# jixinya/EAMM

Hardware: AMD Instinct MI355X
Metric: 256x256 frames/sec (dense-motion + generator forward) (higher is better)
Workload: dtype f32; 1 GPU; 256x256, 10 keypoints, batch=16 synthetic frames per GPU per step, source encoded once per clip (BASELINE.json configs[2]); parallelism=frame-sharded x1

## Files before the change

eamm_amd/csrc/api_common.h:

```cpp
#pragma once
#include "../../include/eamm_hip.h"
#include "kernels.h"

#include <algorithm>
#include <cmath>
#include <cstdarg>
#include <cstdio>
#include <cstdlib>
#include <cstring>
#include <map>
#include <string>
#include <vector>

namespace eamm {

inline thread_local std::string g_create_error;

namespace {

struct HostTensor {
    std::vector<int64_t> shape;
    std::vector<float> data;
    size_t numel() const {
        size_t n = 1;
// ... 170 lines not shown

enum LayerMode { MODE_PLAIN = 0, MODE_PHASE = 1, MODE_ROWSPLIT = 2, MODE_PHASES = 3 };

int upload_bias(CtxBase* c, float** dst, const std::vector<float>& b, size_t n) {
    std::vector<float> pad(n, 0.f);
    std::copy(b.begin(), b.end(), pad.begin());
    return upload(c, dst, pad);
}

int upload_conv_image(CtxBase* c, float** dst, const HostConv& f, const int* map, int cin_packed, int BN, LayerMode mode,
                      bool swizzle) {
    const bool phase = mode == MODE_PHASE || mode == MODE_PHASES;
    std::vector<float> packed(conv_packed_elems(phase ? 4 : f.kh * f.kw, cin_packed, f.Cout, BN, phase ? 4 : 1));
    if (mode == MODE_PHASES)
        conv_pack_phases_host(f.w.data(), f.Cout, f.Cin, map, cin_packed, BN, swizzle, packed.data());
    else
        conv_pack_host(f.w.data(), f.Cout, f.Cin, f.kh, f.kw, map, cin_packed, BN, phase, swizzle, packed.data());
    return upload(c, dst, packed);
}

int pack_conv(CtxBase* c, const HostConv& f, const int* map, int C0_packed, int C1_packed, LayerMode mode, int dma_cfg,
              ConvLayer* L, int BN = 0) {
    const bool phase = mode == MODE_PHASE || mode == MODE_PHASES;
    L->kh = f.kh;
    L->kw = f.kw;
    L->phase = phase;
    L->C0 = C0_packed;
    L->C1 = C1_packed;
    L->Cout = f.Cout;
    L->BM = 128;
    L->BN = BN ? BN : conv_tile_n(f.Cout);
    L->dma_cfg = dma_cfg;
    if (dma_cfg > 0 && !conv_dma_tile(dma_cfg, &L->BM, &L->BN)) return fail(c, EAMM_ERR_ARG, "unknown dma tile %d", dma_cfg);
    L->ntiles = (f.Cout + L->BN - 1) / L->BN;
    L->nchunks = (phase ? 4 : f.kh * f.kw) * ((C0_packed + C1_packed) / CONV_BK);
    if (int rc = upload_conv_image(c, &L->w, f, map, C0_packed + C1_packed, L->BN, mode, dma_cfg > 0)) return rc;
    return upload_bias(c, &L->bias, f.b, (size_t)L->ntiles * L->BN);
}

int pack_patch(CtxBase* c, const HostConv& f, const int* map, int C0_packed, int C1_packed, bool poly, PatchLayer* P) {
    const int cin_packed = C0_packed + C1_packed;
    P->C0 = C0_packed;
    P->C1 = C1_packed;
    P->Cout = f.Cout;
    std::vector<float> packed(poly ? patch_poly_packed_elems(cin_packed, f.Cout) : patch_packed_elems(cin_packed, f.Cout));
    if (poly)
        patch_poly_pack_host(f.w.data(), f.Cout, f.Cin, map, cin_packed, packed.data());
    else
        patch_pack_host(f.w.data(), f.Cout, f.Cin, map, cin_packed, packed.data());
    if (int rc = upload(c, poly ? &P->w_poly : &P->w, packed)) return rc;
    return upload_bias(c, &P->bias, f.b, (size_t)((f.Cout + 63) / 64) * 64);
}

int pack_wino(CtxBase* c, const HostConv& f, int tile, WinoLayer* L) {
    L->Cin = f.Cin;
    L->Cout = f.Cout;
    L->tile = tile;
    L->BN = tile == 4 ? 64 : 128;
    L->ntiles = (f.Cout + L->BN - 1) / L->BN;
    std::vector<float> packed(tile == 4 ? wino4_packed_elems(f.Cout, f.Cin, L->BN) : wino_packed_elems(f.Cout, f.Cin, L->BN));
    if (tile == 4)
        wino4_pack_host(f.w.data(), f.Cout, f.Cin, L->BN, packed.data());
    else
        wino_pack_host(f.w.data(), f.Cout, f.Cin, L->BN, packed.data());
    if (int rc = upload(c, &L->u, packed)) return rc;
    return upload_bias(c, &L->bias, f.b, (size_t)L->ntiles * L->BN);
}

int build_layer(CtxBase* c, const std::vector<FoldSpec>& parts, int ks, int C0_real, int C0_packed, int C1_real,
                int C1_packed, ConvLayer* L, LayerMode mode = MODE_PLAIN, std::vector<float>* row_bias = nullptr,
                int dma_cfg = 0, float** w_swizzled = nullptr, int w_swizzled_bn = 0) {
    if (mode != MODE_PLAIN && mode != MODE_ROWSPLIT) return fail(c, EAMM_ERR_ARG, "build_layer: plain or row-split layers only");
    HostConv f;
    if (int rc = fold_conv(c, parts, ks, C0_real + C1_real, &f)) return rc;
    if (mode == MODE_ROWSPLIT) {
        std::vector<float> rb = to_rowsplit(&f);
        if (row_bias) row_bias->swap(rb);
    }
    const std::vector<int> map = channel_map(C0_real, C0_packed, C1_real, C1_packed);
    if (int rc = pack_conv(c, f, map.data(), C0_packed, C1_packed, MODE_PLAIN, dma_cfg, L)) return rc;
    if (!w_swizzled) return EAMM_OK;
    return upload_conv_image(c, w_swizzled, f, map.data(), C0_packed + C1_packed, w_swizzled_bn ? w_swizzled_bn : L->BN,
                             MODE_PLAIN, true);
}

int build_set(CtxBase* c, const std::vector<FoldSpec>& parts, int C0_real, int C0_packed, int C1_real, int C1_packed,
              LayerSet* S, LayerMode mode) {
    HostConv f;
    int rc = fold_conv(c, parts, 3, C0_real + C1_real, &f);
    if (rc) return rc;
    const std::vector<int> map = channel_map(C0_real, C0_packed, C1_real, C1_packed);
    if ((rc = pack_conv(c, f, map.data(), C0_packed, C1_packed, mode, 0, &S->base))) return rc;
    const int Cout = S->base.Cout;
    int cfg = 0;
    if (Cout % 256 == 0) cfg = c->dma_cfg_n256;
    else if (Cout % 128 == 0) cfg = c->dma_cfg_n128;
    else if (Cout == 64) cfg = c->dma_cfg_n64;
    if (cfg > 0 && c->dma_min_m >= 0) {
        if ((rc = pack_conv(c, f, map.data(), C0_packed, C1_packed, mode, cfg, &S->dma))) return rc;
        S->has_dma = true;
        if (S->dma.BN == 128 && c->skinny_max_m > 0) {
            S->skinny32 = S->dma;
            S->skinny64 = S->dma;
            S->skinny32.dma_cfg = 4;
            S->skinny64.dma_cfg = 5;
            conv_dma_tile(4, &S->skinny32.BM, &S->skinny32.BN);
            conv_dma_tile(5, &S->skinny64.BM, &S->skinny64.BN);
            S->has_skinny = true;
        }
        if (Cout % 256 == 0 && cfg != 1 && c->big_min_m >= 0) {
            if ((rc = pack_conv(c, f, map.data(), C0_packed, C1_packed, mode, 1, &S->big))) return rc;
            S->has_big = true;
        }
    }
    if (mode == MODE_PHASE && parts.size() == 1 && !parts[0].norm.empty() && (Cout & 3) == 0 && c->patch_min_blocks >= 0) {
        if ((rc = pack_patch(c, f, map.data(), C0_packed, C1_packed, c->patch_poly != 0, &S->patch))) return rc;
        S->has_patch = true;
    }
    return 0;
}

size_t set_partial_elems(const LayerSet& S, size_t M) {
    size_t n = conv_plan(S.base, (int)M).partial_elems;
    if (S.has_dma) n = std::max(n, conv_plan(S.dma, (int)M).partial_elems);
    if (S.has_big) n = std::max(n, conv_plan(S.big, (int)M).partial_elems);
    if (S.has_skinny) n = std::max({n, conv_plan(S.skinny32, (int)M).partial_elems, conv_plan(S.skinny64, (int)M).partial_elems});
    return n;
}

int build_wino(CtxBase* c, const std::string& conv, const std::string& norm, int C, WinoLayer* L, int tile = 2) {
    HostConv f;
    if (int rc = fold_conv(c, {{conv, norm}}, 3, C, &f)) return rc;
    if (f.Cout != C) return fail(c, EAMM_ERR_KEY, "%s mis-shaped for the Winograd path", conv.c_str());
    return pack_wino(c, f, tile, L);
}

int build_wino4_rect(CtxBase* c, const std::string& conv, const std::string& norm, int Cin_real, int Cin_packed, WinoLayer* L) {
    if (Cin_packed < Cin_real || Cin_packed % 64) return fail(c, EAMM_ERR_KEY, "%s mis-shaped for the Winograd path", conv.c_str());
    HostConv f;
    if (int rc = fold_conv(c, {{conv, norm}}, 3, Cin_real, &f)) return rc;
    HostConv p = f;
    p.Cin = Cin_packed;
    p.w.assign((size_t)f.Cout * Cin_packed * 9, 0.f);
    for (int o = 0; o < f.Cout; ++o)
        std::copy_n(f.w.begin() + (size_t)o * Cin_real * 9, (size_t)Cin_real * 9, p.w.begin() + (size_t)o * Cin_packed * 9);
    return pack_wino(c, p, 4, L);
}

const ConvLayer& pick(const CtxBase* c, const LayerSet& S, size_t M) {
    if (S.has_skinny && M <= (size_t)c->skinny_max_m) return M <= 32 ? S.skinny32 : S.skinny64;
    if (S.has_big && M >= (size_t)c->big_min_m) return S.big;
    return (S.has_dma && M >= (size_t)c->dma_min_m) ? S.dma : S.base;
}

int launch_up(CtxBase* c, const LayerSet& S, const ConvIO& io, hipStream_t s) {
    if (S.has_patch) {
        int cus = 256;
        (void)hipDeviceGetAttribute(&cus, hipDeviceAttributeMultiprocessorCount, c->device);
        int splits = 1;
        if (S.patch.w_poly) {
            splits = patch_poly_splits(S.patch, io.B, io.Hin, io.Win, c->patch_split_max, cus);
            if ((size_t)splits * io.B * 4 * io.Hin * io.Win * S.patch.Cout > io.partial_cap) splits = 1;
        }
        const int blocks = ((io.Hin + 15) / 16) * ((io.Win + 15) / 16) * io.B * ((S.patch.Cout + 31) / 32) * splits;
        if (blocks >= c->patch_min_blocks && io.Hin >= 16 && io.Win >= 16 && io.act == ACT_RELU && !io.resid && !io.out2 && !io.pool && !io.nchw) {
            if (S.patch.w_poly)
                HIP_TRY(c, patch_poly_launch(S.patch, io.in0, io.in1, io.B, io.Hin, io.Win, io.act, io.out, s, splits, io.partial,
                                             io.partial_cap));
            else
                HIP_TRY(c, patch_phase_launch(S.patch, io.in0, io.in1, io.B, io.Hin, io.Win, io.act, io.out, s));
            return EAMM_OK;
        }
    }
    HIP_TRY(c, conv_launch(pick(c, S, (size_t)io.B * io.Hin * io.Win), io, s));
    return EAMM_OK;
}

int env_int(const char* name, int dflt) { return (int)knob_int(name, dflt); }

int round_up(int v, int m) { return (v + m - 1) / m * m; }

bool is_pow2(int v) { return v > 0 && (v & (v - 1)) == 0; }


inline void read_tile_knobs(CtxBase* c) {
    c->dma_min_m = env_int("EAMM_DMA_MIN_M", c->dma_min_m);
    c->big_min_m = env_int("EAMM_BIG_MIN_M", c->big_min_m);
    c->patch_poly = env_int("EAMM_PATCH_POLY", c->patch_poly);
    c->dma_cfg_n256 = env_int("EAMM_DMA_CFG_N256", c->dma_cfg_n256);
    c->dma_cfg_n128 = env_int("EAMM_DMA_CFG_N128", c->dma_cfg_n128);
    c->dma_cfg_n64 = env_int("EAMM_DMA_CFG_N64", c->dma_cfg_n64);
    c->patch_min_blocks = env_int("EAMM_PATCH_MIN_BLOCKS", c->patch_min_blocks);
    c->patch_split_max = env_int("EAMM_PATCH_SPLIT_MAX", c->patch_split_max);
    c->skinny_max_m = env_int("EAMM_SKINNY_MAX_M", c->skinny_max_m);
}

inline void free_owned(CtxBase* c) {
    DeviceGuard guard(c->device);
    (void)hipDeviceSynchronize();
// ... 38 lines not shown
```

eamm_amd/csrc/conv_winograd4.hip:

```cpp
#include "conv_common.h"

#include <algorithm>
#include <cstdlib>

namespace eamm {

typedef __attribute__((address_space(3))) void* lds_ptr_t;
typedef float f32x4_t __attribute__((ext_vector_type(4)));

template <int VEC> struct vec_of;
template <> struct vec_of<1> { typedef float type; };
template <> struct vec_of<2> { typedef float type __attribute__((ext_vector_type(2))); };
template <> struct vec_of<4> { typedef float type __attribute__((ext_vector_type(4))); };

template <typename T> __device__ __forceinline__ T vfma(float a, T x, T y);
template <> __device__ __forceinline__ float vfma<float>(float a, float x, float y) { return fmaf(a, x, y); }
template <> __device__ __forceinline__ vec_of<2>::type vfma(float a, vec_of<2>::type x, vec_of<2>::type y) {
    vec_of<2>::type r;
    r[0] = fmaf(a, x[0], y[0]); r[1] = fmaf(a, x[1], y[1]);
    return r;
}
template <> __device__ __forceinline__ vec_of<4>::type vfma(float a, vec_of<4>::type x, vec_of<4>::type y) {
    vec_of<4>::type r;
    r[0] = fmaf(a, x[0], y[0]); r[1] = fmaf(a, x[1], y[1]); r[2] = fmaf(a, x[2], y[2]); r[3] = fmaf(a, x[3], y[3]);
    return r;
}
template <typename T> __device__ __forceinline__ T vrelu_affine(T v, T sc, T sh);
template <> __device__ __forceinline__ float vrelu_affine<float>(float v, float sc, float sh) { return fmaxf(fmaf(v, sc, sh), 0.f); }
template <> __device__ __forceinline__ vec_of<2>::type vrelu_affine(vec_of<2>::type v, vec_of<2>::type sc, vec_of<2>::type sh) {
    vec_of<2>::type r;
    r[0] = fmaxf(fmaf(v[0], sc[0], sh[0]), 0.f); r[1] = fmaxf(fmaf(v[1], sc[1], sh[1]), 0.f);
    return r;
}
template <> __device__ __forceinline__ vec_of<4>::type vrelu_affine(vec_of<4>::type v, vec_of<4>::type sc, vec_of<4>::type sh) {
    vec_of<4>::type r;
    r[0] = fmaxf(fmaf(v[0], sc[0], sh[0]), 0.f); r[1] = fmaxf(fmaf(v[1], sc[1], sh[1]), 0.f);
    r[2] = fmaxf(fmaf(v[2], sc[2], sh[2]), 0.f); r[3] = fmaxf(fmaf(v[3], sc[3], sh[3]), 0.f);
    return r;
}

template <typename T> __device__ __forceinline__ void bt6(T& d0, T& d1, T& d2, T& d3, T& d4, T& d5) {
    const T s12 = d1 + d2, m12 = d1 - d2;
    const T s34 = d3 + d4, m43 = d4 - d3;
    const T m31 = d3 - d1, m42 = d4 - d2;
    const T t0 = vfma(4.f, d0, vfma(-5.f, d2, d4));
    const T t1 = vfma(-4.f, s12, s34);
    const T t2 = vfma(4.f, m12, m43);
    const T t3 = vfma(2.f, m31, m42);
    const T t4 = vfma(-2.f, m31, m42);
    const T t5 = vfma(4.f, d1, vfma(-5.f, d3, d5));
    d0 = t0; d1 = t1; d2 = t2; d3 = t3; d4 = t4; d5 = t5;
}

template <int VEC>
__global__ __launch_bounds__(256) void wino4_input_transform_kernel(const float* __restrict__ x,
                                                                    const float* __restrict__ s,
// ... 34 lines not shown
            for (int j = 0; j < 6; ++j) d[i][j] = img[(size_t)(yo[i] + xo[j]) * cvn];
#pragma unroll
        for (int i = 0; i < 6; ++i)
#pragma unroll
            for (int j = 0; j < 6; ++j) {
                T v = d[i][j];
                if (s != nullptr) v = vrelu_affine(v, sc, sh);
                d[i][j] = (oky[i] && okx[j]) ? v : T(0.f);
            }
#pragma unroll
        for (int j = 0; j < 6; ++j) bt6(d[0][j], d[1][j], d[2][j], d[3][j], d[4][j], d[5][j]);
        T* out = reinterpret_cast<T*>(V) + q * cvn + cv;
        const size_t plane = Mq * cvn;
#pragma unroll
        for (int i = 0; i < 6; ++i) {
            bt6(d[i][0], d[i][1], d[i][2], d[i][3], d[i][4], d[i][5]);
            if constexpr (VEC == 4) {
                if (by_xcd & 2) {
                    const __amdgpu_buffer_rsrc_t rs = __builtin_amdgcn_make_buffer_rsrc((void*)V, 0, (unsigned)(36 * plane * 16), 0x00020000);
#pragma unroll
                    for (int j = 0; j < 6; ++j)
                        __builtin_amdgcn_raw_buffer_store_b128(__builtin_bit_cast(u32x4, d[i][j]), rs,
                                                               (unsigned)(((size_t)(i * 6 + j) * plane + q * cvn + cv) * 16), 0, 2);
                    continue;
                }
            }
#pragma unroll
            for (int j = 0; j < 6; ++j) out[(size_t)(i * 6 + j) * plane] = d[i][j];
        }
    }
}

struct Wino4Args {
    const float* V;
    const float* U;
    const float* bias;
    unsigned v_bytes, u_bytes;
    int Mq, C, Cout;
    int H, W;
    int mtiles, ntiles;
    int act;
    const float* resid;
    float* out;
    int groups;
    float* zout;
    float* epi_scratch;
};

__constant__ float WINO4_AT[4][8] = {{1.f, 1.f, 1.f, 1.f, 1.f, 0.f, 0.f, 0.f},
                                     {0.f, 1.f, -1.f, 2.f, -2.f, 0.f, 0.f, 0.f},
                                     {0.f, 1.f, 1.f, 4.f, 4.f, 0.f, 0.f, 0.f},
                                     {0.f, 1.f, -1.f, 8.f, -8.f, 1.f, 0.f, 0.f}};

template <int NT, int WM, int WN, int SUB, int NST, int PE, int DBG = 0>
__global__ __launch_bounds__(WM* WN * 64) void wino4_gemm_kernel(const Wino4Args p) {
    constexpr int NW = WM * WN, NTHR = NW * 64;
    constexpr int BM = WM * 16, BN = WN * NT * 16, BK = CONV_BK;
    constexpr int A_STAGE = SUB * BM * BK, B_STAGE = SUB * BN * BK;
    constexpr int A_INSTR = BM / 8 / NW, B_INSTR = BN / 8 / NW;
    constexpr int NPIECE = SUB * (A_INSTR + B_INSTR);
    constexpr bool TRACE = DBG == 8 || DBG == 9;
    static_assert(BM % (8 * NW) == 0 && BN % (8 * NW) == 0, "tile rows must split evenly over the waves");
    static_assert(BK == 32, "two 16-wide K steps per chunk");

    extern __shared__ __attribute__((aligned(16))) float smem[];
    float* const As = smem;
    float* const Bs = smem + NST * A_STAGE;

    const int tid = threadIdx.x;
    const int lane = tid & 63;
    const int wave = __builtin_amdgcn_readfirstlane(tid >> 6);
    const int r16 = lane & 15, g = lane >> 4;
    const int wm = wave / WN, wn = wave % WN;

    const int L = xcd_remap(blockIdx.x, gridDim.x);
    const int ntile = L % p.ntiles;
    const int mtile = (L / p.ntiles) % p.mtiles;
    const int grp = L / (p.ntiles * p.mtiles);
    const int xis_per = 36 / p.groups;
    const int xi0 = grp * xis_per;
    const int mbase = mtile * BM;
    const int cchunks = p.C / BK;
    const int ci_base = xi0 * cchunks;
    const int nsuper = xis_per * cchunks / SUB;

    unsigned arow_off[A_INSTR];
#pragma unroll
    for (int j = 0; j < A_INSTR; ++j) {
        const int row = (wave * A_INSTR + j) * 8 + (lane >> 3);
        const int slot = (lane & 7) ^ ((row >> 1) & 7);
        const int m = mbase + row;
        arow_off[j] = m < p.Mq ? (unsigned)(m * p.C + slot * 4) * 4u : 0xFFFFF000u;
    }
    const unsigned b_lane = (unsigned)lane * 16u;
    const __amdgpu_buffer_rsrc_t rsv = __builtin_amdgcn_make_buffer_rsrc((void*)p.V, 0, p.v_bytes, 0x00020000);
    const __amdgpu_buffer_rsrc_t rsu = __builtin_amdgcn_make_buffer_rsrc((void*)p.U, 0, p.u_bytes, 0x00020000);
    const unsigned plane_bytes = (unsigned)p.Mq * (unsigned)p.C * 4u;
    const unsigned a_wrap = plane_bytes - (unsigned)(cchunks * BK * 4);

    unsigned sa_off = (unsigned)xi0 * plane_bytes;
    unsigned sb_off = (unsigned)((ntile * 36 * cchunks + ci_base) * BN * BK) * 4u +
                      (unsigned)(wave * B_INSTR * 8 * BK) * 4u;
    int dma_cc = 0, n_st = 0;
    auto dma_advance = [&]() {
        dma_cc += SUB;
        sa_off += SUB * BK * 4;
        if (dma_cc == cchunks) {
            dma_cc = 0;
            sa_off += a_wrap;
        }
        sb_off += SUB * BN * BK * 4;
        n_st = n_st + 1 == NST ? 0 : n_st + 1;
    };
    auto dma_piece = [&](auto kc) {
        constexpr int k = decltype(kc)::value;
        constexpr int sub = k / (A_INSTR + B_INSTR), r = k % (A_INSTR + B_INSTR);
        if constexpr (r < A_INSTR) {
            float* dst = As + n_st * A_STAGE + sub * (BM * BK) + (wave * A_INSTR + r) * (8 * BK) - sub * BK;
            const unsigned vo = arow_off[r];
            __builtin_amdgcn_raw_ptr_buffer_load_lds(rsv, (lds_ptr_t)dst, 16, vo, sa_off, sub * BK * 4, DBG == 40 ? 2 : 0);
        } else {
            constexpr int j = r - A_INSTR;
            float* dst = Bs + n_st * B_STAGE + sub * (BN * BK) + (wave * B_INSTR + j) * (8 * BK);
            __builtin_amdgcn_raw_ptr_buffer_load_lds(rsu, (lds_ptr_t)dst, 16, b_lane,
                                                     sb_off + (unsigned)((sub * BN + j * 8) * BK * 4), 0, 0);
        }
    };

    f32x4_t acc[NT];
    f32x4_t Z[4][NT];
    f32x4_t Y[16][NT];
    static_for<NT>([&](auto jc) {
        constexpr int j = decltype(jc)::value;
        static_for<4>([&](auto rc) {
            constexpr int r = decltype(rc)::value;
            acc[j][r] = 0.f;
            static_for<4>([&](auto qc) { Z[decltype(qc)::value][j][r] = 0.f; });
            static_for<16>([&](auto pc) { Y[decltype(pc)::value][j][r] = 0.f; });
        });
    });

    const int sw = (r16 >> 1) & 7;
    constexpr int STEPS = SUB * 2;
    constexpr int MF = 4 * NT;
    constexpr int TOTAL_MF = STEPS * MF;
    static_assert(PE >= 1 && NPIECE * PE <= TOTAL_MF, "DMA pieces must fit in the interval");
    auto compute = [&](int st, auto more_c, auto young_c) {
        constexpr bool MORE = decltype(more_c)::value && DBG != 1 && DBG != 9, YOUNG = decltype(young_c)::value;
        f32x4_t a[2], b[2][NT];
        auto fetch = [&](int step, int buf) {
            const int sub = step >> 1, s = step & 1;
            const int slot = ((4 * s + g) ^ sw) << 2;
            const float* a_base = As + st * A_STAGE + sub * (BM * BK) + (wm * 16 + r16) * BK + slot;
            const float* b_base = Bs + st * B_STAGE + sub * (BN * BK) + (wn * NT * 16 + r16) * BK + slot;
            a[buf] = *reinterpret_cast<const f32x4_t*>(a_base);
#pragma unroll
            for (int j = 0; j < NT; ++j) b[buf][j] = *reinterpret_cast<const f32x4_t*>(b_base + j * 16 * BK);
        };
        fetch(0, 0);
        if constexpr (MORE && YOUNG) static_for<NPIECE>([&](auto kc) { dma_piece(kc); });
        static_for<STEPS>([&](auto sc) {
            constexpr int step = decltype(sc)::value;
            if constexpr (step + 1 < STEPS) fetch(step + 1, (step + 1) & 1);
            __builtin_amdgcn_sched_barrier(0);
            static_for<MF>([&](auto qc) {
                constexpr int q = decltype(qc)::value;
                constexpr int t = q / NT, j = q % NT;
                acc[j] = __builtin_amdgcn_mfma_f32_16x16x4f32(a[step & 1][t], b[step & 1][j][t], acc[j], 0, 0, 0);
                constexpr int gi = step * MF + q;
                if constexpr (MORE && !YOUNG && gi % PE == PE - 1 && gi / PE < NPIECE) {
                    __builtin_amdgcn_sched_barrier(0);
                    dma_piece(std::integral_constant<int, gi / PE>{});
                    __builtin_amdgcn_sched_barrier(0);
                }
            });
        });
    };
    const bool young = wave >= NW / 2;
    auto interval = [&](int st, bool more) {
        if (more) {
            if (young) compute(st, std::true_type{}, std::true_type{});
            else compute(st, std::true_type{}, std::false_type{});
            dma_advance();
        } else {
            compute(st, std::false_type{}, std::false_type{});
        }
    };

    auto fold_x = [&](int j) {
        const float c0 = WINO4_AT[0][j], c1 = WINO4_AT[1][j], c2 = WINO4_AT[2][j], c3 = WINO4_AT[3][j];
        static_for<NT>([&](auto jc) {
            constexpr int jj = decltype(jc)::value;
            static_for<4>([&](auto rc) {
                constexpr int r = decltype(rc)::value;
                const float m = acc[jj][r];
                Z[0][jj][r] = fmaf(c0, m, Z[0][jj][r]);
                Z[1][jj][r] = fmaf(c1, m, Z[1][jj][r]);
                Z[2][jj][r] = fmaf(c2, m, Z[2][jj][r]);
                Z[3][jj][r] = fmaf(c3, m, Z[3][jj][r]);
                acc[jj][r] = 0.f;
            });
        });
    };
    auto fold_y = [&](int i) {
        const float c0 = WINO4_AT[0][i], c1 = WINO4_AT[1][i], c2 = WINO4_AT[2][i], c3 = WINO4_AT[3][i];
        static_for<NT>([&](auto jc) {
            constexpr int jj = decltype(jc)::value;
            static_for<4>([&](auto qc) {
                constexpr int q = decltype(qc)::value;
                static_for<4>([&](auto rc) {
                    constexpr int r = decltype(rc)::value;
                    const float z = Z[q][jj][r];
                    Y[0 + q][jj][r] = fmaf(c0, z, Y[0 + q][jj][r]);
                    Y[4 + q][jj][r] = fmaf(c1, z, Y[4 + q][jj][r]);
                    Y[8 + q][jj][r] = fmaf(c2, z, Y[8 + q][jj][r]);
                    Y[12 + q][jj][r] = fmaf(c3, z, Y[12 + q][jj][r]);
                    Z[q][jj][r] = 0.f;
                });
            });
        });
    };

    auto store_z = [&](int i) {
        static_for<4>([&](auto qc) {
            constexpr int q = decltype(qc)::value;
            static_for<NT>([&](auto jc) {
                constexpr int jj = decltype(jc)::value;
                const int col = ntile * BN + wn * NT * 16 + jj * 16 + r16;
                static_for<4>([&](auto rc) {
                    constexpr int r = decltype(rc)::value;
                    const int row = mbase + wm * 16 + 4 * g + r;
                    if (row < p.Mq && col < p.Cout) p.zout[((size_t)(i * 4 + q) * p.Mq + row) * p.Cout + col] = Z[q][jj][r];
                    Z[q][jj][r] = 0.f;
                });
            });
        });
    };

// ... 125 lines not shown
        const int qx = m % Wq, tq = m / Wq;
        const int qy = tq % Hq, b = tq / Hq;
        const f32x4_t* z = reinterpret_cast<const f32x4_t*>(Z) + idx;
        const f32x4_t bs = reinterpret_cast<const f32x4_t*>(bias)[c4];
        const float lo = act == ACT_RELU ? 0.f : -INFINITY;
        f32x4_t colsum[2];
#pragma unroll
        for (int q = 0; q < 4; ++q) {
            f32x4_t zi[6];
#pragma unroll
            for (int i = 0; i < 6; ++i) zi[i] = z[(size_t)(i * 4 + q) * plane];
            const f32x4_t s12 = zi[1] + zi[2], d12 = zi[1] - zi[2], s34 = zi[3] + zi[4], d34 = zi[3] - zi[4];
            f32x4_t y[4];
            y[0] = zi[0] + s12 + s34;
            y[1] = d12 + 2.f * d34;
            y[2] = s12 + 4.f * s34;
            y[3] = d12 + 8.f * d34 + zi[5];
            f32x4_t r4[4];
            if constexpr (RESID) {
#pragma unroll
                for (int pp = 0; pp < 4; ++pp)
                    r4[pp] = reinterpret_cast<const f32x4_t*>(resid)[(((size_t)(b * H + 4 * qy + pp) * W + 4 * qx + q) * Cout) / 4 + c4];
            }
#pragma unroll
            for (int pp = 0; pp < 4; ++pp) {
                f32x4_t v = y[pp] + bs;
                if constexpr (!POOL) {
                    const size_t o = (((size_t)(b * H + 4 * qy + pp) * W + 4 * qx + q) * Cout) / 4 + c4;
                    if constexpr (RESID) v = v + r4[pp];
                    v[0] = fmaxf(v[0], lo); v[1] = fmaxf(v[1], lo); v[2] = fmaxf(v[2], lo); v[3] = fmaxf(v[3], lo);
                    reinterpret_cast<f32x4_t*>(out)[o] = v;
                } else {
                    v[0] = fmaxf(v[0], lo); v[1] = fmaxf(v[1], lo); v[2] = fmaxf(v[2], lo); v[3] = fmaxf(v[3], lo);
                    y[pp] = v;
                }
            }
            if constexpr (POOL) {
                if ((q & 1) == 0) {
                    colsum[0] = y[0] + y[1];
                    colsum[1] = y[2] + y[3];
                } else {
#pragma unroll
                    for (int py = 0; py < 2; ++py) {
                        const f32x4_t v = 0.25f * (colsum[py] + (y[2 * py] + y[2 * py + 1]));
                        const size_t o = (((size_t)(b * (H >> 1) + 2 * qy + py) * (W >> 1) + 2 * qx + (q >> 1)) * Cout) / 4 + c4;
                        reinterpret_cast<f32x4_t*>(out)[o] = v;
                    }
                }
            }
        }
    }
}

void wino4_pack_host(const float* w, int Cout, int Cin, int BN, float* dst) {
    static const double G[6][3] = {{1.0 / 4, 0, 0},           {-1.0 / 6, -1.0 / 6, -1.0 / 6}, {-1.0 / 6, 1.0 / 6, -1.0 / 6},
                                   {1.0 / 24, 1.0 / 12, 1.0 / 6}, {1.0 / 24, -1.0 / 12, 1.0 / 6},  {0, 0, 1}};
    const int BK = CONV_BK, cch = Cin / BK;
    const int ntiles = (Cout + BN - 1) / BN;
    const size_t total = (size_t)ntiles * 36 * cch * BN * BK;
    for (size_t i = 0; i < total; ++i) dst[i] = 0.f;
    for (int o = 0; o < Cout; ++o) {
        const int nt = o / BN, nl = o % BN;
        for (int c = 0; c < Cin; ++c) {
            const float* gw = w + ((size_t)o * Cin + c) * 9;
            double tmp[6][3];
            for (int i = 0; i < 6; ++i)
                for (int k = 0; k < 3; ++k)
                    tmp[i][k] = G[i][0] * gw[0 * 3 + k] + G[i][1] * gw[1 * 3 + k] + G[i][2] * gw[2 * 3 + k];
            const int cc = c / BK, kl = c % BK;
            const int kk = ((((kl >> 2) ^ ((nl >> 1) & 7)) << 2) | (kl & 3));
            for (int i = 0; i < 6; ++i)
                for (int j = 0; j < 6; ++j) {
                    const double u = tmp[i][0] * G[j][0] + tmp[i][1] * G[j][1] + tmp[i][2] * G[j][2];
                    const int xi = i * 6 + j;
                    dst[(((size_t)nt * 36 * cch + (size_t)xi * cch + cc) * BN + nl) * BK + kk] = (float)u;
                }
        }
    }
}

size_t wino4_packed_elems(int Cout, int Cin, int BN) {
    return (size_t)((Cout + BN - 1) / BN) * 36 * (Cin / CONV_BK) * BN * CONV_BK;
}

hipError_t wino4_transform_launch(const float* x, const float* s, const float* t, int B, int H, int W, int C, float* V,
                                  hipStream_t stream) {
    if ((H & 3) || (W & 3) || (C & 3)) return hipErrorInvalidValue;
    static const int vec_env = [] {
        const int v = (int)knob_int("EAMM_WINO4_TR_VEC", 0);
        return (v == 1 || v == 2 || v == 4) ? v : 0;
    }();
    const int vec = vec_env ? vec_env : ((size_t)B * (H / 4) * (W / 4) * (C / 4) <= 64 * 256 ? 1 : 4);
    const size_t total = (size_t)B * (H / 4) * (W / 4) * (C / vec);
    const int blocks = (int)std::min<size_t>((total + 255) / 256, (size_t)1 << 20);
    static const int xcd = (int)knob_int("EAMM_WINO4_TR_XCD", 3);
    const int remap = ((size_t)blocks * 256 >= total ? (xcd & 1) : 0) | ((36.0 * total * 16 < 4.0e9 && vec == 4) ? (xcd & 2) : 0);
    if (vec == 1)
        hipLaunchKernelGGL(wino4_input_transform_kernel<1>, dim3(blocks), dim3(256), 0, stream, x, s, t, B, H, W, C, V, remap);
    else if (vec == 2)
        hipLaunchKernelGGL(wino4_input_transform_kernel<2>, dim3(blocks), dim3(256), 0, stream, x, s, t, B, H, W, C, V, remap);
    else
        hipLaunchKernelGGL(wino4_input_transform_kernel<4>, dim3(blocks), dim3(256), 0, stream, x, s, t, B, H, W, C, V, remap);
    return hipGetLastError();
}

template <int SUB, int NST, int PE, int DBG = 0, int WM = 4>
static hipError_t wino4_launch_variant(const Wino4Args& a, hipStream_t stream) {
    constexpr int NT = 2, WN = 2;
    constexpr int BM = WM * 16, BN = WN * NT * 16;
    constexpr size_t lds_loop = sizeof(float) * NST * SUB * (BM + BN) * CONV_BK;
    constexpr size_t lds_epi = sizeof(float) * 4 * BM * (BN + 4);
    constexpr size_t lds = lds_loop > lds_epi ? lds_loop : lds_epi;
    static_assert(lds <= 160 * 1024, "LDS budget");
    auto kern = wino4_gemm_kernel<NT, WM, WN, SUB, NST, PE, DBG>;
    static lds_once_mask configured{0};
    if (hipError_t e = ensure_dynamic_lds(kern, lds, &configured); e != hipSuccess) return e;
    note_mfma_flops(2.0 * 36.0 * a.mtiles * BM * (double)a.ntiles * BN * a.C);
    hipLaunchKernelGGL(kern, dim3(a.mtiles * a.ntiles * a.groups), dim3(WM * WN * 64), lds, stream, a);
    return hipGetLastError();
}

hipError_t wino4_gemm_launch(const WinoLayer& L, const float* V, int B, int H, int W, int act, const float* resid,
                             float* out, hipStream_t stream, int variant, int groups, float* zbuf, int pool) {
    constexpr int BM = 64, BN = 64;
    if (pool && (groups == 1 || resid != nullptr)) return hipErrorInvalidValue;
    if (L.tile != 4 || L.BN != BN || (L.Cout & 3) || L.Cin % (2 * CONV_BK) || (H & 3) || (W & 3))
        return hipErrorInvalidValue;
    Wino4Args a{};
    a.V = V;
    a.U = L.u;
    a.bias = L.bias;
    a.Mq = B * (H / 4) * (W / 4);
    a.C = L.Cin;
    a.Cout = L.Cout;
    a.H = H;
    a.W = W;
    a.mtiles = (a.Mq + BM - 1) / BM;
    a.ntiles = L.ntiles;
    static const int narrow_max = (int)knob_int("EAMM_WINO4_NARROW_MAX_BLOCKS", 128);
    const bool narrow = groups == 6 && a.mtiles * a.ntiles * groups <= narrow_max && L.Cin % (4 * CONV_BK) == 0;
    if (narrow) a.mtiles = (a.Mq + 31) / 32;
    a.act = act;
    a.resid = resid;
    a.out = out;
    if (groups != 1 && groups != 2 && groups != 3 && groups != 6) return hipErrorInvalidValue;
    if (groups > 1 && zbuf == nullptr) return hipErrorInvalidValue;
    a.groups = groups;
    a.zout = groups > 1 ? zbuf : nullptr;
#ifdef EAMM_EXPERIMENTS
    a.epi_scratch = (variant == 50 && groups == 1) ? zbuf : nullptr;
    if (variant == 50 && a.epi_scratch == nullptr) variant = 3;
#else
    if (variant == 10 || variant == 16 || variant == 17 || variant == 50) return hipErrorInvalidValue;
#endif
    const size_t vb = (size_t)36 * a.Mq * a.C * sizeof(float), ub = wino4_packed_elems(L.Cout, L.Cin, BN) * sizeof(float);
    if (vb >= 0xFFFFF000ull || ub >= 0xFFFFF000ull) return hipErrorInvalidValue;
    a.v_bytes = (unsigned)vb;
    a.u_bytes = (unsigned)ub;
    const bool sub4 = L.Cin % (4 * CONV_BK) == 0;
    hipError_t e = hipErrorInvalidValue;
    if (narrow) variant = 30;
    switch (variant) {
        case 30: e = wino4_launch_variant<4, 2, 4, 0, 2>(a, stream); break;
#ifdef EAMM_EXPERIMENTS
        case 50: e = sub4 ? wino4_launch_variant<4, 2, 8, 30>(a, stream) : wino4_launch_variant<2, 2, 4>(a, stream); break;
        case 10: e = wino4_launch_variant<4, 2, 4, 1>(a, stream); break;
        case 16: e = wino4_launch_variant<4, 2, 4, 8>(a, stream); break;
        case 17: e = wino4_launch_variant<4, 2, 4, 9>(a, stream); break;
#endif
        case 0: e = sub4 ? wino4_launch_variant<4, 2, 4>(a, stream) : wino4_launch_variant<2, 2, 4>(a, stream); break;
        case 3: e = sub4 ? wino4_launch_variant<4, 2, 8>(a, stream) : wino4_launch_variant<2, 2, 4>(a, stream); break;
        case 6: e = sub4 ? wino4_launch_variant<4, 2, 8, 40>(a, stream) : wino4_launch_variant<2, 2, 4>(a, stream); break;
        default: break;
    }
    if (e != hipSuccess || groups == 1) return e;
    const size_t total = (size_t)a.Mq * (L.Cout / 4);
    const int blocks = (int)std::min<size_t>((total + 255) / 256, (size_t)1 << 20);
    if (pool)
        hipLaunchKernelGGL((wino4_output_transform_kernel<true, false>), dim3(blocks), dim3(256), 0, stream, zbuf, L.bias, resid,
                           a.Mq, L.Cout, H, W, act, out);
    else if (resid != nullptr)
        hipLaunchKernelGGL((wino4_output_transform_kernel<false, true>), dim3(blocks), dim3(256), 0, stream, zbuf, L.bias, resid,
                           a.Mq, L.Cout, H, W, act, out);
    else
        hipLaunchKernelGGL((wino4_output_transform_kernel<false, false>), dim3(blocks), dim3(256), 0, stream, zbuf, L.bias, resid,
                           a.Mq, L.Cout, H, W, act, out);
    return hipGetLastError();
}

}
```

eamm_amd/csrc/kernels.h:

```cpp
#pragma once
#include <hip/hip_runtime.h>
#include <stddef.h>
#include <stdint.h>

namespace eamm {

constexpr int CONV_BK = 32;
constexpr int CONV_LDK = CONV_BK + 4;
constexpr int KP_STRIDE = 8;

enum Act { ACT_NONE = 0, ACT_RELU = 1, ACT_SIGMOID = 2 };

void note_mfma_flops(double flops);
double take_mfma_flops();
double total_mfma_flops();

long long knob_int(const char* name, long long dflt);
int knobs_json(char* buf, int cap);

struct ConvArgs {
    const float* in0;
    const float* in1;
    int C0, C1;
    unsigned in0_bytes, in1_bytes, w_bytes;
// ... 35 lines not shown
                    bool phase, bool swizzle, float* dst);
void conv_pack_phases_host(const float* wph, int Cout, int Cin, const int* cin_map, int cin_packed, int BN, bool swizzle,
                           float* dst);
bool conv_dma_tile(int dma_cfg, int* BM, int* BN);
struct ConvArgs;
hipError_t conv_dma_launch_kernel(const ConvLayer& L, const ConvArgs& a, int blocks, hipStream_t stream);

struct ConvPlan {
    int mtiles, ntiles, splits, chunks_per_split, Mpad, Npad;
    size_t partial_elems;
};
ConvPlan conv_plan(const ConvLayer& L, int M, int force_splits = 0);

struct ConvIO {
    const float* in0; const float* in1;
    int B, Hin, Win;
    int act, pool, nchw;
    const float* resid;
    float* out; float* out2; const float* s2; const float* t2;
    float* partial;
    size_t partial_cap;
    int split_n;
};
hipError_t conv_launch(const ConvLayer& L, const ConvIO& io, hipStream_t stream, int force_splits = 0);

struct PatchLayer {
    int C0 = 0, C1 = 0, Cout = 0;
    float* w = nullptr;
    float* w_poly = nullptr;
    float* bias = nullptr;
};
size_t patch_packed_elems(int Cin_packed, int Cout);
size_t patch_poly_packed_elems(int Cin_packed, int Cout);
void patch_poly_pack_host(const float* w_oihw_3x3, int Cout, int Cin, const int* cin_map, int cin_packed, float* dst);
hipError_t patch_poly_launch(const PatchLayer& L, const float* in0, const float* in1, int B, int H, int W, int act,
                             float* out, hipStream_t stream, int splits = 1, float* partial = nullptr, size_t partial_cap = 0);
int patch_poly_splits(const PatchLayer& L, int B, int H, int W, int max_splits, int cus);
void patch_pack_host(const float* w_oihw_3x3, int Cout, int Cin, const int* cin_map, int cin_packed, float* dst);
hipError_t patch_phase_launch(const PatchLayer& L, const float* in0, const float* in1, int B, int H, int W, int act,
                              float* out, hipStream_t stream);

hipError_t conv_col7_launch(const float* in, int C, int B, int H, int W, const float* w_swizzled, float* out,
                            hipStream_t stream);
hipError_t conv_col7_fused_launch(const float* in, int C, int B, int H, int W, const float* w_swizzled, const float* bias,
                                  float* out_nchw, hipStream_t stream);

hipError_t conv_col7s_launch(const float* in0, int C0, const float* in1, int C1, int B, int H, int W, const float* w_swizzled,
                             int ntile32, float* out, int pixel_stride, hipStream_t stream);

struct WinoLayer {
    int Cin = 0, Cout = 0, BN = 128, ntiles = 0;
    int tile = 2;
    float* u = nullptr;
    float* bias = nullptr;
};
size_t wino_packed_elems(int Cout, int Cin, int BN);
void wino_pack_host(const float* w_oihw, int Cout, int Cin, int BN, float* dst);
hipError_t wino_transform_launch(const float* x, const float* s, const float* t, int B, int H, int W, int C, float* V,
                                 hipStream_t stream);
hipError_t wino_gemm_launch(const WinoLayer& L, const float* V, int B, int H, int W, int act, const float* resid,
                            float* out, hipStream_t stream);

size_t wino4_packed_elems(int Cout, int Cin, int BN);
void wino4_pack_host(const float* w_oihw, int Cout, int Cin, int BN, float* dst);
hipError_t wino4_transform_launch(const float* x, const float* s, const float* t, int B, int H, int W, int C, float* V,
                                  hipStream_t stream);
hipError_t wino4_gemm_launch(const WinoLayer& L, const float* V, int B, int H, int W, int act, const float* resid,
                             float* out, hipStream_t stream, int variant = 0, int groups = 1, float* zbuf = nullptr, int pool = 0);

bool first7_supported(int Cout);
void first7_pack_host(const float* w_oihw_7x7_folded, int Cout, float* dst );
hipError_t first7_launch(const float* src , const float* w_packed, const float* bias, int ns, int H, int W,
                         int Cout, float* out , hipStream_t stream);

hipError_t kp_prepare_launch(const float* kd_val, const float* kd_jac, const float* ks_val, const float* ks_jac,
                             int n, int ns, int K, float* kp_rec, int* bad_flag, hipStream_t s);
hipError_t motion_front_launch(const float* kp_rec, const float* src_small , int n, int ns, int K,
                               int h, int w, float variance, int Cpad, float* hg_in ,
                               float* sparse_deformed , hipStream_t s, int groups = 1,
                               int channels = 3, size_t group_stride = 0);
hipError_t motion_head_launch(const float* logits , const float* kp_rec, int n, int K, int h, int w,
                              int has_occ, float* deformation , float* occlusion ,
                              float* mask_out , float* occ_out ,
                              hipStream_t s);
hipError_t motion_head_rowsplit_launch(const float* part , int PS, int NC,
                                       const float* bias , const float* kp_rec, int n, int K, int h, int w,
                                       int has_occ, float* deformation, float* occlusion, float* mask_out,
                                       float* occ_out, hipStream_t s);
hipError_t warp_features_launch(const float* feat , const float* deformation ,
                                const float* occlusion , int n, int ns, int hf, int wf, int C,
                                int h, int w, float* out, float* out2, const float* s2, const float* t2,
                                hipStream_t s);
hipError_t broadcast_features_launch(const float* feat , int n, int ns, int hf, int wf, int C, float* out,
                                     float* out2, const float* s2, const float* t2, hipStream_t s);
hipError_t warp_image_launch(const float* src , const float* deformation , int n, int ns,
                             int H, int W, int h, int w, float* out , hipStream_t s, int src_planes = 3,
                             int channels = 3);
hipError_t source_prepare_launch(const float* src , const float* aa_w , int ns, int H,
                                 int W, int inv_scale, int Cpad, float* src_nhwc ,
                                 float* src_small , hipStream_t s);
hipError_t final_shift_sum_launch(const float* part , const float* bias ,
                                  int n, int H, int W, float* out , hipStream_t s);
hipError_t antialias_down_launch(const float* src , const float* aa_w, int ns, int H, int W,
                                 int inv_scale, int Cpad, float* dst , hipStream_t s,
                                 int src_planes = 3, int first_channel = 0, int channels = 3, int slot = 0);
hipError_t nchw_to_nhwc_pad_launch(const float* src , int B, int C, int H, int W, int Cpad,
                                   float* dst , hipStream_t s, int planes = 0 );
hipError_t kp_head_launch(const float* logits , int B, int K, int njm, int h, int w, int Cs, int pad,
                          float temperature, float* value , float* jacobian ,
                          float* heatmap , hipStream_t s,
                          float* ws = nullptr ,
                          float* stats = nullptr );
constexpr int KP_HEAD_SLICES = 8;
size_t kp_head_workspace_floats(int B, int K);
constexpr int KP_HEAD_BWD_SLICES = 32;
size_t kp_head_backward_workspace_floats(int B, int K);
hipError_t kp_head_backward_launch(const float* logits , const float* stats , const float* value ,
// ... 170 lines not shown
```

Measured before the change: 4041 frames/s.

## Emulate fp32 Winograd-4 GEMM with three-way bf16 split MFMA

Adds a split-precision path to the Winograd F(4,3) GEMM. Each fp32 value is decomposed into three bf16 planes. Weights are pre-split on the host into a lane-ordered 3-plane layout, and activations are split in registers. The product is accumulated with six bf16 16x16x32 MFMA terms per sub-step. This trades the slower fp32 (xf32/f32) MFMA path for faster bf16 MFMAs, at the cost of 1.5x weight bytes per stage, extra split ALU work, and a small accuracy change from truncating the split terms.

Result: faster. 4202 frames/s (median of 6 runs) (+4.0%).

```diff
diff --git a/eamm_amd/csrc/api_common.h b/eamm_amd/csrc/api_common.h
--- a/eamm_amd/csrc/api_common.h
+++ b/eamm_amd/csrc/api_common.h
@@ -246,7 +246,7 @@
     return upload_bias(c, &P->bias, f.b, (size_t)((f.Cout + 63) / 64) * 64);
 }
 
-int pack_wino(CtxBase* c, const HostConv& f, int tile, WinoLayer* L) {
+int pack_wino(CtxBase* c, const HostConv& f, int tile, WinoLayer* L, bool split_planes = true) {
     L->Cin = f.Cin;
     L->Cout = f.Cout;
     L->tile = tile;
@@ -258,6 +258,11 @@
     else
         wino_pack_host(f.w.data(), f.Cout, f.Cin, L->BN, packed.data());
     if (int rc = upload(c, &L->u, packed)) return rc;
+    if (split_planes && tile == 4 && f.Cin % (4 * CONV_BK) == 0) {
+        std::vector<float> planes(wino4_split_packed_elems(f.Cout, f.Cin, L->BN));
+        wino4_pack_split_host(f.w.data(), f.Cout, f.Cin, L->BN, reinterpret_cast<uint16_t*>(planes.data()));
+        if (int rc = upload(c, &L->u3, planes)) return rc;
+    }
     return upload_bias(c, &L->bias, f.b, (size_t)L->ntiles * L->BN);
 }
 
@@ -338,7 +343,7 @@
     p.w.assign((size_t)f.Cout * Cin_packed * 9, 0.f);
     for (int o = 0; o < f.Cout; ++o)
         std::copy_n(f.w.begin() + (size_t)o * Cin_real * 9, (size_t)Cin_real * 9, p.w.begin() + (size_t)o * Cin_packed * 9);
-    return pack_wino(c, p, 4, L);
+    return pack_wino(c, p, 4, L, false);
 }
 
 const ConvLayer& pick(const CtxBase* c, const LayerSet& S, size_t M) {
diff --git a/eamm_amd/csrc/conv_winograd4.hip b/eamm_amd/csrc/conv_winograd4.hip
--- a/eamm_amd/csrc/conv_winograd4.hip
+++ b/eamm_amd/csrc/conv_winograd4.hip
@@ -1,7 +1,9 @@
 #include "conv_common.h"
 
 #include <algorithm>
+#include <cstdint>
 #include <cstdlib>
+#include <cstring>
 
 namespace eamm {
 
@@ -142,13 +144,38 @@
                                      {0.f, 1.f, 1.f, 4.f, 4.f, 0.f, 0.f, 0.f},
                                      {0.f, 1.f, -1.f, 8.f, -8.f, 1.f, 0.f, 0.f}};
 
-template <int NT, int WM, int WN, int SUB, int NST, int PE, int DBG = 0>
+typedef __bf16 bf16x8_t __attribute__((ext_vector_type(8)));
+
+__device__ __forceinline__ unsigned wino4_hi_pair(unsigned lo, unsigned hi) { return __builtin_amdgcn_perm(hi, lo, 0x07060302u); }
+
+__device__ __forceinline__ void wino4_split3(const f32x4_t& x0, const f32x4_t& x1, u32x4 (&pl)[3]) {
+#pragma unroll
+    for (int i = 0; i < 4; ++i) {
+        unsigned b1[2], b2[2], b3[2];
+#pragma unroll
+        for (int h = 0; h < 2; ++h) {
+            const float x = i < 2 ? x0[2 * i + h] : x1[2 * i - 4 + h];
+            b1[h] = __float_as_uint(x);
+            const float r = x - __uint_as_float(b1[h] & 0xFFFF0000u);
+            b2[h] = __float_as_uint(r);
+            b3[h] = __float_as_uint(r - __uint_as_float(b2[h] & 0xFFFF0000u));
+        }
+        pl[0][i] = wino4_hi_pair(b1[0], b1[1]);
+        pl[1][i] = wino4_hi_pair(b2[0], b2[1]);
+        pl[2][i] = wino4_hi_pair(b3[0], b3[1]);
+    }
+}
+
+template <int NT, int WM, int WN, int SUB, int NST, int PE, int DBG = 0, int SPLIT = 0>
 __global__ __launch_bounds__(WM* WN * 64) void wino4_gemm_kernel(const Wino4Args p) {
     constexpr int NW = WM * WN, NTHR = NW * 64;
     constexpr int BM = WM * 16, BN = WN * NT * 16, BK = CONV_BK;
-    constexpr int A_STAGE = SUB * BM * BK, B_STAGE = SUB * BN * BK;
+    constexpr int B_CHUNK = SPLIT ? BN * BK * 3 / 2 : BN * BK;
+    constexpr int A_STAGE = SUB * BM * BK, B_STAGE = SUB * B_CHUNK;
     constexpr int A_INSTR = BM / 8 / NW, B_INSTR = BN / 8 / NW;
-    constexpr int NPIECE = SUB * (A_INSTR + B_INSTR);
+    constexpr int U_INSTR = SUB * B_CHUNK / 256 / NW;
+    constexpr int NPIECE = SPLIT ? SUB * A_INSTR + U_INSTR : SUB * (A_INSTR + B_INSTR);
+    static_assert(!SPLIT || (SUB * B_CHUNK) % (256 * NW) == 0, "the stage's U must split evenly into 1 KB pieces per wave");
     constexpr bool TRACE = DBG == 8 || DBG == 9;
     static_assert(BM % (8 * NW) == 0 && BN % (8 * NW) == 0, "tile rows must split evenly over the waves");
     static_assert(BK == 32, "two 16-wide K steps per chunk");
@@ -189,8 +216,8 @@
     const unsigned a_wrap = plane_bytes - (unsigned)(cchunks * BK * 4);
 
     unsigned sa_off = (unsigned)xi0 * plane_bytes;
-    unsigned sb_off = (unsigned)((ntile * 36 * cchunks + ci_base) * BN * BK) * 4u +
-                      (unsigned)(wave * B_INSTR * 8 * BK) * 4u;
+    unsigned sb_off = (unsigned)((ntile * 36 * cchunks + ci_base) * B_CHUNK) * 4u +
+                      (unsigned)(wave * (SPLIT ? U_INSTR * 256 : B_INSTR * 8 * BK)) * 4u;
     int dma_cc = 0, n_st = 0;
     auto dma_advance = [&]() {
         dma_cc += SUB;
@@ -199,16 +226,21 @@
             dma_cc = 0;
             sa_off += a_wrap;
         }
-        sb_off += SUB * BN * BK * 4;
+        sb_off += SUB * B_CHUNK * 4;
         n_st = n_st + 1 == NST ? 0 : n_st + 1;
     };
     auto dma_piece = [&](auto kc) {
         constexpr int k = decltype(kc)::value;
-        constexpr int sub = k / (A_INSTR + B_INSTR), r = k % (A_INSTR + B_INSTR);
+        constexpr int sub = SPLIT ? (k < SUB * A_INSTR ? k / A_INSTR : 0) : k / (A_INSTR + B_INSTR);
+        constexpr int r = SPLIT ? (k < SUB * A_INSTR ? k % A_INSTR : A_INSTR + k - SUB * A_INSTR) : k % (A_INSTR + B_INSTR);
         if constexpr (r < A_INSTR) {
             float* dst = As + n_st * A_STAGE + sub * (BM * BK) + (wave * A_INSTR + r) * (8 * BK) - sub * BK;
             const unsigned vo = arow_off[r];
             __builtin_amdgcn_raw_ptr_buffer_load_lds(rsv, (lds_ptr_t)dst, 16, vo, sa_off, sub * BK * 4, DBG == 40 ? 2 : 0);
+        } else if constexpr (SPLIT) {
+            constexpr int j = r - A_INSTR;
+            float* dst = Bs + n_st * B_STAGE + (wave * U_INSTR + j) * 256;
+            __builtin_amdgcn_raw_ptr_buffer_load_lds(rsu, (lds_ptr_t)dst, 16, b_lane, sb_off + (unsigned)(j * 1024), 0, 0);
         } else {
             constexpr int j = r - A_INSTR;
             float* dst = Bs + n_st * B_STAGE + sub * (BN * BK) + (wave * B_INSTR + j) * (8 * BK);
@@ -233,7 +265,8 @@
     const int sw = (r16 >> 1) & 7;
     constexpr int STEPS = SUB * 2;
     constexpr int MF = 4 * NT;
-    constexpr int TOTAL_MF = STEPS * MF;
+    constexpr int MF_SPLIT = 6 * NT;
+    constexpr int TOTAL_MF = SPLIT ? SUB * MF_SPLIT : STEPS * MF;
     static_assert(PE >= 1 && NPIECE * PE <= TOTAL_MF, "DMA pieces must fit in the interval");
     auto compute = [&](int st, auto more_c, auto young_c) {
         constexpr bool MORE = decltype(more_c)::value && DBG != 1 && DBG != 9, YOUNG = decltype(young_c)::value;
@@ -266,14 +299,73 @@
             });
         });
     };
+    auto compute_split = [&](int st, auto more_c, auto young_c) {
+        constexpr bool MORE = decltype(more_c)::value && DBG != 1 && DBG != 9, YOUNG = decltype(young_c)::value;
+        f32x4_t araw[2];
+        u32x4 ap[3], ub[3][NT];
+        auto fetch_a = [&](int sub) {
+            const float* a_base = As + st * A_STAGE + sub * (BM * BK) + (wm * 16 + r16) * BK;
+            araw[0] = *reinterpret_cast<const f32x4_t*>(a_base + ((g ^ sw) << 2));
+            araw[1] = *reinterpret_cast<const f32x4_t*>(a_base + (((4 + g) ^ sw) << 2));
+        };
+        auto fetch_u = [&](int sub, int pl) {
+            const float* u_base = Bs + st * B_STAGE + sub * B_CHUNK + ((wn * NT) * 3 + pl) * 256 + lane * 4;
+#pragma unroll
+            for (int j = 0; j < NT; ++j) ub[pl][j] = *reinterpret_cast<const u32x4*>(u_base + j * 3 * 256);
+        };
+        auto term = [&](auto sc, auto tc) {
+            constexpr int sub = decltype(sc)::value, t = decltype(tc)::value;
+            constexpr int pa = t == 0 ? 0 : t == 1 ? 2 : t == 2 ? 1 : t == 3 ? 0 : t == 4 ? 1 : 0;
+            constexpr int pb = t == 0 ? 2 : t <= 3 ? 0 : 1;
+            static_for<NT>([&](auto jc) {
+                constexpr int j = decltype(jc)::value;
+                acc[j] = __builtin_amdgcn_mfma_f32_16x16x32_bf16(__builtin_bit_cast(bf16x8_t, ap[pa]), __builtin_bit_cast(bf16x8_t, ub[pb][j]),
+                                                                  acc[j], 0, 0, 0);
+                constexpr int gi = sub * MF_SPLIT + t * NT + j;
+                if constexpr (MORE && !YOUNG && gi % PE == PE - 1 && gi / PE < NPIECE) {
+                    __builtin_amdgcn_sched_barrier(0);
+                    dma_piece(std::integral_constant<int, gi / PE>{});
+                    __builtin_amdgcn_sched_barrier(0);
+                }
+            });
+        };
+        fetch_a(0);
+        if constexpr (MORE && YOUNG) static_for<NPIECE>([&](auto kc) { dma_piece(kc); });
+        static_for<SUB>([&](auto sc) {
+            constexpr int sub = decltype(sc)::value;
+            fetch_u(sub, 2);
+            __builtin_amdgcn_sched_barrier(0);
+            wino4_split3(araw[0], araw[1], ap);
+            __builtin_amdgcn_sched_barrier(0);
+            fetch_u(sub, 0);
+            __builtin_amdgcn_sched_barrier(0);
+            term(sc, std::integral_constant<int, 0>{});
+            __builtin_amdgcn_sched_barrier(0);
+            fetch_u(sub, 1);
+            __builtin_amdgcn_sched_barrier(0);
+            term(sc, std::integral_constant<int, 1>{});
+            term(sc, std::integral_constant<int, 2>{});
+            term(sc, std::integral_constant<int, 3>{});
+            __builtin_amdgcn_sched_barrier(0);
+            if constexpr (sub + 1 < SUB) fetch_a(sub + 1);
+            __builtin_amdgcn_sched_barrier(0);
+            term(sc, std::integral_constant<int, 4>{});
+            term(sc, std::integral_constant<int, 5>{});
+            __builtin_amdgcn_sched_barrier(0);
+        });
+    };
     const bool young = wave >= NW / 2;
+    auto run = [&](int st, auto more_c, auto young_c) {
+        if constexpr (SPLIT) compute_split(st, more_c, young_c);
+        else compute(st, more_c, young_c);
+    };
     auto interval = [&](int st, bool more) {
         if (more) {
-            if (young) compute(st, std::true_type{}, std::true_type{});
-            else compute(st, std::true_type{}, std::false_type{});
+            if (young) run(st, std::true_type{}, std::true_type{});
+            else run(st, std::true_type{}, std::false_type{});
             dma_advance();
         } else {
-            compute(st, std::false_type{}, std::false_type{});
+            run(st, std::false_type{}, std::false_type{});
         }
     };
 
@@ -505,36 +597,63 @@
     }
 }
 
-void wino4_pack_host(const float* w, int Cout, int Cin, int BN, float* dst) {
+namespace {
+template <typename F>
+void wino4_for_each_u(const float* w, int Cout, int Cin, F&& put) {
     static const double G[6][3] = {{1.0 / 4, 0, 0},           {-1.0 / 6, -1.0 / 6, -1.0 / 6}, {-1.0 / 6, 1.0 / 6, -1.0 / 6},
                                    {1.0 / 24, 1.0 / 12, 1.0 / 6}, {1.0 / 24, -1.0 / 12, 1.0 / 6},  {0, 0, 1}};
-    const int BK = CONV_BK, cch = Cin / BK;
-    const int ntiles = (Cout + BN - 1) / BN;
-    const size_t total = (size_t)ntiles * 36 * cch * BN * BK;
-    for (size_t i = 0; i < total; ++i) dst[i] = 0.f;
     for (int o = 0; o < Cout; ++o) {
-        const int nt = o / BN, nl = o % BN;
         for (int c = 0; c < Cin; ++c) {
             const float* gw = w + ((size_t)o * Cin + c) * 9;
             double tmp[6][3];
             for (int i = 0; i < 6; ++i)
                 for (int k = 0; k < 3; ++k)
                     tmp[i][k] = G[i][0] * gw[0 * 3 + k] + G[i][1] * gw[1 * 3 + k] + G[i][2] * gw[2 * 3 + k];
-            const int cc = c / BK, kl = c % BK;
-            const int kk = ((((kl >> 2) ^ ((nl >> 1) & 7)) << 2) | (kl & 3));
             for (int i = 0; i < 6; ++i)
                 for (int j = 0; j < 6; ++j) {
                     const double u = tmp[i][0] * G[j][0] + tmp[i][1] * G[j][1] + tmp[i][2] * G[j][2];
-                    const int xi = i * 6 + j;
-                    dst[(((size_t)nt * 36 * cch + (size_t)xi * cch + cc) * BN + nl) * BK + kk] = (float)u;
+                    put(o, c, i * 6 + j, (float)u);
                 }
         }
     }
+}
+}
+
+void wino4_pack_host(const float* w, int Cout, int Cin, int BN, float* dst) {
+    const int BK = CONV_BK, cch = Cin / BK;
+    const size_t total = wino4_packed_elems(Cout, Cin, BN);
+    for (size_t i = 0; i < total; ++i) dst[i] = 0.f;
+    wino4_for_each_u(w, Cout, Cin, [&](int o, int c, int xi, float u) {
+        const int nt = o / BN, nl = o % BN;
+        const int cc = c / BK, kl = c % BK;
+        const int kk = ((((kl >> 2) ^ ((nl >> 1) & 7)) << 2) | (kl & 3));
+        dst[(((size_t)nt * 36 * cch + (size_t)xi * cch + cc) * BN + nl) * BK + kk] = u;
+    });
 }
 
 size_t wino4_packed_elems(int Cout, int Cin, int BN) {
     return (size_t)((Cout + BN - 1) / BN) * 36 * (Cin / CONV_BK) * BN * CONV_BK;
 }
+
+void wino4_pack_split_host(const float* w, int Cout, int Cin, int BN, uint16_t* dst) {
+    const int BK = CONV_BK, cch = Cin / BK;
+    const size_t total = 3 * wino4_packed_elems(Cout, Cin, BN);
+    for (size_t i = 0; i < total; ++i) dst[i] = 0;
+    auto bits = [](float f) { uint32_t b; memcpy(&b, &f, 4); return b; };
+    auto top = [](uint32_t b) { b &= 0xFFFF0000u; float f; memcpy(&f, &b, 4); return f; };
+    wino4_for_each_u(w, Cout, Cin, [&](int o, int c, int xi, float u) {
+        const int nt = o / BN, nl = o % BN;
+        const int cc = c / BK, kl = c % BK;
+        const int lane = ((kl & 15) >> 2) * 16 + (nl & 15), e = (kl >> 4) * 4 + (kl & 3);
+        const float r = u - top(bits(u)), r2 = r - top(bits(r));
+        uint16_t* blk = dst + ((((size_t)nt * 36 * cch + (size_t)xi * cch + cc) * (BN / 16) + nl / 16) * 3) * 512 + lane * 8 + e;
+        blk[0] = (uint16_t)(bits(u) >> 16);
+        blk[512] = (uint16_t)(bits(r) >> 16);
+        blk[1024] = (uint16_t)(bits(r2) >> 16);
+    });
+}
+
+size_t wino4_split_packed_elems(int Cout, int Cin, int BN) { return wino4_packed_elems(Cout, Cin, BN) * 3 / 2; }
 
 hipError_t wino4_transform_launch(const float* x, const float* s, const float* t, int B, int H, int W, int C, float* V,
                                   hipStream_t stream) {
@@ -557,15 +676,15 @@
     return hipGetLastError();
 }
 
-template <int SUB, int NST, int PE, int DBG = 0, int WM = 4>
+template <int SUB, int NST, int PE, int DBG = 0, int WM = 4, int SPLIT = 0>
 static hipError_t wino4_launch_variant(const Wino4Args& a, hipStream_t stream) {
     constexpr int NT = 2, WN = 2;
     constexpr int BM = WM * 16, BN = WN * NT * 16;
-    constexpr size_t lds_loop = sizeof(float) * NST * SUB * (BM + BN) * CONV_BK;
+    constexpr size_t lds_loop = sizeof(float) * NST * SUB * (BM + (SPLIT ? BN * 3 / 2 : BN)) * CONV_BK;
     constexpr size_t lds_epi = sizeof(float) * 4 * BM * (BN + 4);
     constexpr size_t lds = lds_loop > lds_epi ? lds_loop : lds_epi;
     static_assert(lds <= 160 * 1024, "LDS budget");
-    auto kern = wino4_gemm_kernel<NT, WM, WN, SUB, NST, PE, DBG>;
+    auto kern = wino4_gemm_kernel<NT, WM, WN, SUB, NST, PE, DBG, SPLIT>;
     static lds_once_mask configured{0};
     if (hipError_t e = ensure_dynamic_lds(kern, lds, &configured); e != hipSuccess) return e;
     note_mfma_flops(2.0 * 36.0 * a.mtiles * BM * (double)a.ntiles * BN * a.C);
@@ -606,11 +725,14 @@
 #else
     if (variant == 10 || variant == 16 || variant == 17 || variant == 50) return hipErrorInvalidValue;
 #endif
-    const size_t vb = (size_t)36 * a.Mq * a.C * sizeof(float), ub = wino4_packed_elems(L.Cout, L.Cin, BN) * sizeof(float);
+    const bool sub4 = L.Cin % (4 * CONV_BK) == 0;
+    const bool split = groups == 1 && sub4 && L.u3 != nullptr && (variant == 3 || variant == 6);
+    if (split) a.U = L.u3;
+    const size_t vb = (size_t)36 * a.Mq * a.C * sizeof(float),
+                 ub = (split ? wino4_split_packed_elems(L.Cout, L.Cin, BN) : wino4_packed_elems(L.Cout, L.Cin, BN)) * sizeof(float);
     if (vb >= 0xFFFFF000ull || ub >= 0xFFFFF000ull) return hipErrorInvalidValue;
     a.v_bytes = (unsigned)vb;
     a.u_bytes = (unsigned)ub;
-    const bool sub4 = L.Cin % (4 * CONV_BK) == 0;
     hipError_t e = hipErrorInvalidValue;
     if (narrow) variant = 30;
     switch (variant) {
@@ -622,8 +744,8 @@
         case 17: e = wino4_launch_variant<4, 2, 4, 9>(a, stream); break;
 #endif
         case 0: e = sub4 ? wino4_launch_variant<4, 2, 4>(a, stream) : wino4_launch_variant<2, 2, 4>(a, stream); break;
-        case 3: e = sub4 ? wino4_launch_variant<4, 2, 8>(a, stream) : wino4_launch_variant<2, 2, 4>(a, stream); break;
-        case 6: e = sub4 ? wino4_launch_variant<4, 2, 8, 40>(a, stream) : wino4_launch_variant<2, 2, 4>(a, stream); break;
+        case 3: e = split ? wino4_launch_variant<4, 2, 4, 0, 4, 1>(a, stream) : sub4 ? wino4_launch_variant<4, 2, 8>(a, stream) : wino4_launch_variant<2, 2, 4>(a, stream); break;
+        case 6: e = split ? wino4_launch_variant<4, 2, 4, 40, 4, 1>(a, stream) : sub4 ? wino4_launch_variant<4, 2, 8, 40>(a, stream) : wino4_launch_variant<2, 2, 4>(a, stream); break;
         default: break;
     }
     if (e != hipSuccess || groups == 1) return e;
diff --git a/eamm_amd/csrc/kernels.h b/eamm_amd/csrc/kernels.h
--- a/eamm_amd/csrc/kernels.h
+++ b/eamm_amd/csrc/kernels.h
@@ -111,6 +111,7 @@
     int Cin = 0, Cout = 0, BN = 128, ntiles = 0;
     int tile = 2;
     float* u = nullptr;
+    float* u3 = nullptr;
     float* bias = nullptr;
 };
 size_t wino_packed_elems(int Cout, int Cin, int BN);
@@ -122,6 +123,8 @@
 
 size_t wino4_packed_elems(int Cout, int Cin, int BN);
 void wino4_pack_host(const float* w_oihw, int Cout, int Cin, int BN, float* dst);
+size_t wino4_split_packed_elems(int Cout, int Cin, int BN);
+void wino4_pack_split_host(const float* w_oihw, int Cout, int Cin, int BN, uint16_t* dst);
 hipError_t wino4_transform_launch(const float* x, const float* s, const float* t, int B, int H, int W, int C, float* V,
                                   hipStream_t stream);
 hipError_t wino4_gemm_launch(const WinoLayer& L, const float* V, int B, int H, int W, int act, const float* resid,
```
